# ruiminshen/yolo-tf

Measured on AMD Instinct MI355X. Metric: train_throughput, higher is better.
Workload: dtype bf16; 1 GPU; Darknet-19 YOLOv2 VOC-20 416x416 training step (standardise+fwd+loss+bwd+Adam), batch 16 per GPU (BASELINE configs[1]); global_batch=16, parallelism=dp1, optimizer=adam, weights=random-init (Xavier, seed 0), collective=none (1 rank)

## Files before the change

include/yolo2_hip.h:

```cpp
#ifndef YOLO2_HIP_H
#define YOLO2_HIP_H

#include <stddef.h>
#include <stdint.h>

#ifdef __cplusplus
extern "C" {
#endif

enum { YOLO2_F32 = 0, YOLO2_BF16 = 1 };
enum {
    YOLO2_OK = 0,
    YOLO2_E_ARG = 1,
    YOLO2_E_LAUNCH = 2,
    YOLO2_E_UNSUPPORTED = 3
};

int yolo2_abi_version(void);
const char *yolo2_last_error(void);
uint32_t yolo2_crc32c(const void *data, size_t n, uint32_t crc);
int yolo2_shutdown(void);
int yolo2_check_async_errors(void *stream);
#define YOLO2_ASYNC_ERROR_WORDS 8
int yolo2_async_error_snapshot(unsigned *host_words, void *stream);
// ... 24 lines not shown
int yolo2_conv2d_wgrad_ws(const void *X, const void *dY, float *dW, float *ws, size_t ws_bytes, int B, int H, int W,
                          int Cin, int ldx, int Cout, int ldy, int ksize, int dtype, void *stream);
int yolo2_set_deterministic(int on);
int yolo2_get_deterministic(void);

int yolo2_filter_prep(const float *W, void *Ffwd, void *Fdgr, int ksize, int Cin, int ldcin,
                      int Cout, int ldcout, int dtype, void *stream);

#define YOLO2_FILTER_PREP_TILE 64
#define YOLO2_FILTER_PREP_TILE_N 128
int yolo2_filter_prep_blocks(int ksize, int ldcin, int ldcout);
typedef struct yolo2_filter_desc {
    const float *W;
    void *Ffwd;
    void *Fdgr;
    int ksize, cin, ldcin, cout, ldcout, first_block;
} yolo2_filter_desc;
int yolo2_filter_prep_batch(const yolo2_filter_desc *descs_device, int n, int total_blocks, int dtype,
                            void *stream);

int yolo2_adam_filter_prep(const yolo2_filter_desc *descs_device, int n, int total_blocks, const long *small_ranges_device, int n_small,
                           float *params, const float *grads, float *m, float *v, float alpha, float beta1, float beta2, float eps,
                           float gscale, int dtype, void *stream);

int yolo2_conv2d_bias_leaky(const void *P, const void *F, const float *bias, void *O, float *ws, size_t ws_bytes, int B,
                            int H, int W, int Cp, int ldp, int Nf, int ldo, int ksize, float alpha, int dtype, void *stream);

int yolo2_conv2d_dgrad_bn(const void *dY, const void *F, void *dX, float *ws, size_t ws_bytes, int B, int H, int W, int Cp, int ldp,
                          int Nf, int ldo, int ksize, const void *Yprev, const float *mean, const float *var, const float *gamma,
                          const float *beta, float *dgamma, float *dbeta, float *bn_part, double *red_ws, float eps, float alpha,
                          int *pending, int dtype, void *stream);
int yolo2_conv2d_dgrad_bn_fuses(int B, int H, int W, int Nf, int ksize, int dtype);
int yolo2_bn_part_to_grads(float *bn_part, int C, float *dgamma, float *dbeta, void *stream);

#define YOLO2_BN_PART_ROWS 256
int yolo2_conv2d_bn(const void *P, const void *F, void *O, float *ws, size_t ws_bytes, int B, int H, int W, int Cp, int ldp,
                    int Nf, int ldo, int ksize, const float *shift, float *bn_part, int dtype, void *stream);
int yolo2_bn_finalize(float *bn_part, const float *shift, long M, int C, float *mean, float *var, float *moving_mean,
                      float *moving_var, double decay, void *stream);

int yolo2_last_bn_part_rows(void);
int yolo2_bn_fin_supported(int rows, int C, int dtype);
int yolo2_bn_leaky_fin(const void *Y, const float *bn_part, int rows, const float *shift, float *mean, float *var, float *moving_mean,
                       float *moving_var, double decay, const float *gamma, const float *beta, void *A, long M, int C, int lda,
                       float eps, float alpha, float *zero, long zero_floats, int dtype, void *stream);
int yolo2_bn_leaky_pool_fin(const void *Y, const float *bn_part, int rows, const float *shift, float *mean, float *var,
// ... 202 lines not shown
```

yolo_tf_amd/_lib.py:

```python
import ctypes
import os

_HERE = os.path.dirname(os.path.abspath(__file__))
LIB_PATH = os.environ.get('YOLO2_LIB_PATH') or os.path.join(_HERE, 'csrc', 'libyolo2hip.so')

F32, BF16 = 0, 1


class HipKernelError(RuntimeError):
    pass


_p = ctypes.c_void_p
_i = ctypes.c_int
_l = ctypes.c_long
_f = ctypes.c_float

SIGNATURES = {
    'yolo2_conv2d': [_p, _p, _p, _p, _i, _i, _i, _i, _i, _i, _i, _i, _i, _p],
    'yolo2_conv2d_ws': [_p, _p, _p, _p, _p, ctypes.c_size_t, _i, _i, _i, _i, _i, _i, _i, _i, _i, _p],
    'yolo2_conv2d_bias_leaky': [_p, _p, _p, _p, _p, ctypes.c_size_t, _i, _i, _i, _i, _i, _i, _i, _i, _f, _i, _p],
    'yolo2_conv2d_dgrad_bn': [_p, _p, _p, _p, ctypes.c_size_t, _i, _i, _i, _i, _i, _i, _i, _i, _p, _p, _p, _p, _p, _p, _p, _p, _p, _f, _f, _p, _i, _p],
    'yolo2_bn_part_to_grads': [_p, _i, _p, _p, _p],
    'yolo2_debug_noop': [_p],
    'yolo2_conv2d_wgrad': [_p, _p, _p, _i, _i, _i, _i, _i, _i, _i, _i, _i, _p],
    'yolo2_conv2d_wgrad_ws': [_p, _p, _p, _p, ctypes.c_size_t, _i, _i, _i, _i, _i, _i, _i, _i, _i, _p],
    'yolo2_set_deterministic': [_i],
    'yolo2_filter_prep': [_p, _p, _p, _i, _i, _i, _i, _i, _i, _p],
    'yolo2_filter_prep_batch': [_p, _i, _i, _i, _p],
    'yolo2_adam_filter_prep': [_p, _i, _i, _p, _i, _p, _p, _p, _p, _f, _f, _f, _f, _f, _i, _p],
    'yolo2_first_layer_stats': [_p, _p, _i, _i, _i, _p, _p, _i, _p],
    'yolo2_first_layer_bn_leaky_pool': [_p, _p, _p, _p, _p, _p, _p, _p, _i, _i, _i, _i, _f, _f, _i, _p],
    'yolo2_first_layer_pool_bwd_reduce': [_p, _p, _p, _i, _p, _p, _p, _p, _p, _p, _i, _i, _i, _f, _f, _i, _p],
    'yolo2_first_layer_pool_bwd_apply': [_p, _p, _p, _i, _p, _p, _p, _p, _p, _p, _p, _p, _i, _i, _i, _f, _f, _i, _p],
    'yolo2_conv2d_bn': [_p, _p, _p, _p, ctypes.c_size_t, _i, _i, _i, _i, _i, _i, _i, _i, _p, _p, _i, _p],
    'yolo2_bn_finalize': [_p, _p, _l, _i, _p, _p, _p, _p, ctypes.c_double, _p],
    'yolo2_bn_leaky_fin': [_p, _p, _i, _p, _p, _p, _p, _p, ctypes.c_double, _p, _p, _p, _l, _i, _i, _f, _f, _p, _l, _i, _p],
    'yolo2_bn_leaky_pool_fin': [_p, _p, _i, _p, _p, _p, _p, _p, ctypes.c_double, _p, _p, _p, _p, _p, _p, _i, _i, _i, _i, _i, _f, _f, _p, _l, _i, _p],
    'yolo2_bn_leaky_bwd_apply_fin': [_p, _i, _p, _p, _p, _p, _p, _p, _i, _l, _p, _p, _p, _l, _i, _f, _f, _p, _l, _i, _p],
    'yolo2_first_layer_wgrad_bn': [_p, _p, _p, _i, _p, _p, _p, _p, _p, _p, _i, _l, _p, _p, _p, _i, _i, _i, _i, _f, _f, _p, _l, _i, _p],
    'yolo2_bn_leaky_pool_bwd_apply_fin': [_p, _i, _p, _p, _p, _p, _p, _p, _p, _i, _l, _p, _p, _p, _i, _i, _i, _i, _f, _f, _p, _l, _i, _p],
    'yolo2_bn_leaky_bwd_reduce_part': [_p, _i, _p, _p, _p, _p, _p, _p, _p, _i, _l, _i, _f, _f, _i, _p],
    'yolo2_bn_leaky_pool_bwd_reduce_part': [_p, _i, _p, _p, _p, _p, _p, _p, _p, _p, _i, _i, _i, _i, _i, _f, _f, _i, _p],
    'yolo2_bn_leaky_pool': [_p, _p, _p, _p, _p, _p, _p, _i, _i, _i, _i, _i, _f, _f, _i, _p],
    'yolo2_bn_leaky_pool_bwd_reduce': [_p, _i, _p, _p, _p, _p, _p, _p, _p, _p, _p, _i, _i, _i, _i, _f, _f, _i, _p],
    'yolo2_bn_leaky_pool_bwd_apply': [_p, _i, _p, _p, _p, _p, _p, _p, _p, _p, _p, _i, _i, _i, _i, _f, _f, _i, _p],
    'yolo2_augment_images': [_p, _p, _p, _p, _i, _i, _i, _i, _p],
    'yolo2_transform_labels': [_p, _p, _p, _p, _p, _p, _p, _p, _p, _i, _i, _i, _i, _p, _p],
    'yolo2_bn_stats': [_p, _p, _p, _p, _l, _i, _i, _p],
    'yolo2_bn_stats_ema': [_p, _p, _p, _p, _p, ctypes.c_double, _p, _l, _i, _i, _p],
    'yolo2_bn_ema': [_p, _p, _p, _p, _i, ctypes.c_double, _p],
    'yolo2_bn_leaky': [_p, _p, _p, _p, _p, _p, _l, _i, _i, _f, _f, _i, _p],
    'yolo2_bn_leaky_bwd_reduce': [_p, _i, _p, _p, _p, _p, _p, _p, _p, _p, _l, _i, _f, _f, _i, _p],
# ... 30 lines not shown
    'yolo2_ftrl': [_p, _p, _p, _p, _l, _f, _f, _f, _f, _f, _p],
    'yolo2_scale': [_p, _l, _f, _p],
    'yolo2_zero_ranges': [_p, _p, _i, _p],
    'yolo2_bn_fold': [_p, _p, _p, _p, _p, _p, _p, _l, _i, _f, _p],
    'yolo2_selftest_tr16': [_p, _p],
    'yolo2_set_stream_workgroups': [_i],
    'yolo2_cast_f32_bf16': [_p, _p, _l, _p],
    'yolo2_cast_bf16_f32': [_p, _p, _l, _p],
    'yolo2_debug_occupy': [_i, _p, _p, _i, _p],
    'yolo2_check_async_errors': [_p],
    'yolo2_async_error_snapshot': [_p, _p],
    'yolo2_debug_set_streamk_wait_us': [_i, _i],
    'yolo2_eval_collect': [_p, _p, _p, _p, _p, _p, _p, _i, _i, _i, _i, _i, _i, _i, _f, _f, _p, _l, _p, _p, _p, _p],
    'yolo2_eval_finalize': [_p, _l, _p, _p, _i, _i, _i, _p, ctypes.c_size_t, _p, _p, _p, _p, _p],
}

QUERIES = {
    'yolo2_abi_version': (_i, []),
    'yolo2_last_error': (ctypes.c_char_p, []),
    'yolo2_shutdown': (_i, []),
    'yolo2_crc32c': (ctypes.c_uint32, [_p, ctypes.c_size_t, ctypes.c_uint32]),
    'yolo2_conv2d_wgrad_accumulates': (_i, [_i] * 9),
    'yolo2_filter_prep_blocks': (_i, [_i, _i, _i]),
    'yolo2_conv2d_dgrad_bn_fuses': (_i, [_i] * 6),
    'yolo2_debug_set_wgrad_variant': (None, [_i]),
    'yolo2_last_bn_part_rows': (_i, []),
    'yolo2_get_stream_workgroups': (_i, []),
    'yolo2_bn_fin_supported': (_i, [_i, _i, _i]),
    'yolo2_debug_last_conv_plan': (_i, [ctypes.POINTER(_i)]),
    'yolo2_debug_set_igemm_tap': (_i, [_i]),
    'yolo2_debug_set_pp': (_i, [_i, _i, _i, _i]),
    'yolo2_debug_set_pp_cost': (_i, [_i]),
    'yolo2_debug_set_s4_abl': (_i, [_i]),
    'yolo2_debug_last_wgrad_plan': (_i, [ctypes.POINTER(_i)]),
    'yolo2_debug_wgrad_row_plan': (_i, [_i, _i, _i, _i, _i, _i, _i, ctypes.POINTER(_i)]),
    'yolo2_debug_wgrad_ws_plan': (_i, [_i] * 10 + [ctypes.POINTER(_i)]),
    'yolo2_conv2d_wgrad_workspace_bytes': (ctypes.c_size_t, [_i] * 9),
    'yolo2_get_deterministic': (_i, []),
    'yolo2_debug_magic_u32': (_i, [ctypes.c_uint, ctypes.POINTER(ctypes.c_uint), ctypes.POINTER(ctypes.c_uint)]),
    'yolo2_conv2d_workspace_bytes': (ctypes.c_size_t, [_i] * 7),
    'yolo2_bn_workspace_bytes': (ctypes.c_size_t, [_i]),
    'yolo2_bias_grad_workspace_bytes': (ctypes.c_size_t, [_i]),
    'yolo2_image_prep_workspace_bytes': (ctypes.c_size_t, [_i]),
    'yolo2_loss_workspace_bytes': (ctypes.c_size_t, [_i, _i, _i]),
    'yolo2_nms_workspace_bytes': (ctypes.c_size_t, [_i, _i, _i]),
    'yolo2_clip_workspace_bytes': (ctypes.c_size_t, [_i]),
# ... 104 lines not shown
```

yolo_tf_amd/csrc/elementwise.hip:

```cpp
#include "common.h"
#include <stdlib.h>
#include <stdarg.h>

static thread_local char g_err[512] = "";
void yolo2_set_error(const char *fmt, ...) {
    va_list ap;
    va_start(ap, fmt);
    vsnprintf(g_err, sizeof(g_err), fmt, ap);
    va_end(ap);
}
extern "C" const char *yolo2_last_error(void) { return g_err; }

static thread_local int g_deterministic = 0;
int y2_deterministic() { return g_deterministic; }
extern "C" int yolo2_set_deterministic(int on) { g_deterministic = on ? 1 : 0; return YOLO2_OK; }
extern "C" int yolo2_get_deterministic(void) { return g_deterministic; }

extern "C" uint32_t yolo2_crc32c(const void *data, size_t n, uint32_t crc) {
    static uint32_t table[8][256];
    static bool ready = [] {
        for (uint32_t i = 0; i < 256; ++i) {
            uint32_t c = i;
            for (int k = 0; k < 8; ++k) c = (c & 1) ? (c >> 1) ^ 0x82F63B78u : c >> 1;
            table[0][i] = c;
// ... 50 lines not shown
    }
}

extern "C" int yolo2_filter_prep(const float *W, void *Ffwd, void *Fdgr, int ksize, int Cin, int ldcin,
                                 int Cout, int ldcout, int dtype, void *stream) {
    Y2_CHECK_ARG(W && (Ffwd || Fdgr));
    Y2_CHECK_ARG(ksize == 1 || ksize == 3);
    Y2_CHECK_ARG(ldcin >= Cin && ldcout >= Cout);
    hipStream_t st = (hipStream_t)stream;
    const int taps = ksize * ksize;
    if (Ffwd) {
        dim3 grid(cdiv(Cout, 32), cdiv(ldcin, 32), taps), block(32, 8);
        Y2_DISPATCH_DTYPE(dtype, filter_fwd_kernel<T><<<grid, block, 0, st>>>(W, (T *)Ffwd, Cin, ldcin, Cout, taps));
    }
    if (Fdgr) {
        long total = (long)Cin * taps * ldcout;
        int grid = (int)(total / 256 + 1 < 4096 ? total / 256 + 1 : 4096);
        Y2_DISPATCH_DTYPE(dtype, filter_dgrad_kernel<T><<<grid, 256, 0, st>>>(W, (T *)Fdgr, Cin, Cout, ldcout, taps));
    }
    Y2_CHECK_LAUNCH();
    return YOLO2_OK;
}

template <typename T>
__device__ __forceinline__ void store8(T *dst, const float (&v)[8]) {
    if constexpr (sizeof(T) == 2) {
        bf16x8 o;
#pragma unroll
        for (int j = 0; j < 8; ++j) o[j] = (bf16)v[j];
        *reinterpret_cast<bf16x8 *>(dst) = o;
    } else {
        f32x4 a = {v[0], v[1], v[2], v[3]}, b = {v[4], v[5], v[6], v[7]};
        reinterpret_cast<f32x4 *>(dst)[0] = a;
        reinterpret_cast<f32x4 *>(dst)[1] = b;
    }
}
template <typename T>
__device__ __forceinline__ void filter_tile_emit(const yolo2_filter_desc &d, const float (&tile)[YOLO2_FILTER_PREP_TILE][YOLO2_FILTER_PREP_TILE_N + 1], int tap, int taps,
                                                 int c0, int n0, int tid) {
    constexpr int TC = YOLO2_FILTER_PREP_TILE, TN = YOLO2_FILTER_PREP_TILE_N;
    T *Ff = (T *)d.Ffwd, *Fd = (T *)d.Fdgr;
    if (Ff) {
        constexpr int LPR = TC / 8, RPP = 256 / LPR;
        const int g8 = (tid % LPR) * 8, rr = tid / LPR;
        const long Kf = (long)taps * d.ldcin;
#pragma unroll
        for (int p = 0; p < TN / RPP; ++p) {
            const int nl = rr + p * RPP, nn = n0 + nl, c = c0 + g8;
            if (nn < d.cout && c < d.ldcin) {
                float v[8];
#pragma unroll
                for (int j = 0; j < 8; ++j) v[j] = tile[g8 + j][nl];
                store8<T>(Ff + nn * Kf + y2_filter_koff(tap, c, d.ldcin, taps), v);
            }
        }
    }
    if (Fd) {
        constexpr int LPR = TN / 8, RPP = 256 / LPR;
        const int g8 = (tid % LPR) * 8, rr = tid / LPR;
        const long Kd = (long)taps * d.ldcout;
        const int tp = taps - 1 - tap;
#pragma unroll
        for (int p = 0; p < TC / RPP; ++p) {
            const int cl = rr + p * RPP, c = c0 + cl, nn = n0 + g8;
// ... 1897 lines not shown
    if ((int)blockIdx.x >= conv_blocks) {
        const long *r = small + 2 * ((int)blockIdx.x - conv_blocks);
        for (long k = threadIdx.x; k < r[1]; k += 256) {
            const long o = r[0] + k;
            adam_one(a.params[o], a.grads[o], a.m[o], a.v[o], a.alpha, a.omb1, a.omb2, a.eps, a.gs);
        }
        return;
    }
    constexpr int TC = YOLO2_FILTER_PREP_TILE, TN = YOLO2_FILTER_PREP_TILE_N;
    __shared__ float tile[TC][TN + 1];
    int li = 0;
    while (li + 1 < n && (int)blockIdx.x >= descs[li + 1].first_block) ++li;
    const yolo2_filter_desc d = descs[li];
    const int taps = d.ksize * d.ksize;
    const int ctiles = (d.ldcin + TC - 1) / TC, ntiles = (d.ldcout + TN - 1) / TN;
    int u = blockIdx.x - d.first_block;
    const int ntile = u % ntiles; u /= ntiles;
    const int ctile = u % ctiles;
    const int tap = u / ctiles;
    const int n0 = ntile * TN, c0 = ctile * TC;
    const int tid = threadIdx.x;
    const long base = (d.W - a.params) + (long)tap * d.cin * d.cout;
    const bool vec_ok = (d.cout & 3) == 0 && ((base & 3) == 0);
    {
        constexpr int LPR = TN / 4, RPP = 256 / LPR;
        const int col = (tid % LPR) * 4, r0 = tid / LPR;
#pragma unroll
        for (int p = 0; p < TC / RPP; ++p) {
            const int c = c0 + r0 + p * RPP, nn = n0 + col;
            float w4[4] = {0.f, 0.f, 0.f, 0.f};
            if (c < d.cin) {
                const long o = base + (long)c * d.cout + nn;
                if (vec_ok && nn + 3 < d.cout) {
                    f32x4 wv = *reinterpret_cast<const f32x4 *>(a.params + o), mv = *reinterpret_cast<const f32x4 *>(a.m + o), vv = *reinterpret_cast<const f32x4 *>(a.v + o);
                    const f32x4 gv = *reinterpret_cast<const f32x4 *>(a.grads + o);
#pragma unroll
                    for (int j = 0; j < 4; ++j) {
                        float wj = wv[j], mj = mv[j], vj = vv[j];
                        adam_one(wj, gv[j], mj, vj, a.alpha, a.omb1, a.omb2, a.eps, a.gs);
                        wv[j] = wj; mv[j] = mj; vv[j] = vj; w4[j] = wj;
                    }
                    *reinterpret_cast<f32x4 *>(a.m + o) = mv;
                    *reinterpret_cast<f32x4 *>(a.v + o) = vv;
                    *reinterpret_cast<f32x4 *>(a.params + o) = wv;
                } else {
#pragma unroll
                    for (int j = 0; j < 4; ++j)
// ... 1 lines not shown
                            adam_one(a.params[o + j], a.grads[o + j], a.m[o + j], a.v[o + j], a.alpha, a.omb1, a.omb2, a.eps, a.gs);
                            w4[j] = a.params[o + j];
                        }
                }
            }
#pragma unroll
            for (int j = 0; j < 4; ++j) tile[r0 + p * RPP][col + j] = w4[j];
        }
    }
    __syncthreads();
    filter_tile_emit<T>(d, tile, tap, taps, c0, n0, tid);
}
extern "C" int yolo2_adam_filter_prep(const yolo2_filter_desc *descs_device, int n, int total_blocks, const long *small_ranges_device, int n_small,
                                      float *params, const float *grads, float *m, float *v, float alpha, float beta1, float beta2, float eps,
                                      float gscale, int dtype, void *stream) {
    Y2_CHECK_ARG(n >= 0 && total_blocks >= 0 && (n > 0) == (total_blocks > 0) && (descs_device || n == 0) && n_small >= 0 && total_blocks + n_small > 0 &&
                 (small_ranges_device || n_small == 0) && params && grads && m && v);
    Y2_CHECK_ARG(((((uintptr_t)params) | ((uintptr_t)grads) | ((uintptr_t)m) | ((uintptr_t)v)) & 15) == 0);
    const Y2AdamArgs a{params, grads, m, v, alpha, 1.0f - beta1, 1.0f - beta2, eps, gscale};
    Y2_DISPATCH_DTYPE(dtype, adam_filter_prep_kernel<T><<<total_blocks + n_small, 256, 0, (hipStream_t)stream>>>(descs_device, n, total_blocks, small_ranges_device, a));
    Y2_CHECK_LAUNCH();
    return YOLO2_OK;
}
```

yolo_tf_amd/engine.py:

```python
import numpy as np
import os

import torch

from . import ops, _lib
from .graph import pad8

BN_EPS = 1e-5
BN_DECAY = 0.999
LEAKY_ALPHA = 0.1

_DTYPES = {'bf16': torch.bfloat16, 'bfloat16': torch.bfloat16, 'f32': torch.float32, 'float32': torch.float32}


BN_PART_ROWS = 256
ARENA_ALIGN = 64


def layout_params(graph):
    offsets, off = {}, 0
    for v in reversed(graph.trainable()):
        offsets[v.name] = (off, v.size)
        off += (v.size + ARENA_ALIGN - 1) // ARENA_ALIGN * ARENA_ALIGN
    return offsets, off
# ... 349 lines not shown
        first = 0
        for d, op in zip(arr, convs):
            st = self.conv[op['name']]
            k, ldcin, ldcout = op['ksize'], pad8(op['cin']), pad8(op['cout'])
            if self._folds(op):
                st['fold_w'] = torch.empty_like(self.var[op['weights'].name])
                st['fold_bias'] = torch.empty(op['cout'], dtype=torch.float32, device=self.device)
            d.W = (st['fold_w'] if 'fold_w' in st else self.var[op['weights'].name]).data_ptr()
            d.Ffwd = st['Ffwd'].data_ptr()
            d.Fdgr = st['Fdgr'].data_ptr() if 'Fdgr' in st else None
            d.ksize, d.cin, d.ldcin, d.cout, d.ldcout, d.first_block = k, op['cin'], ldcin, op['cout'], ldcout, first
            first += ops.filter_prep_blocks(k, ldcin, ldcout)
        raw = bytes(arr)
        self._fdesc = torch.frombuffer(bytearray(raw), dtype=torch.uint8).to(self.device)
        self._fdesc_n, self._fdesc_blocks = len(convs), first
        import ctypes
        self._fdesc1_info = {}
        size = ctypes.sizeof(FilterDesc)
        bounds = [d.first_block for d in arr] + [first]
        for i, (d, op) in enumerate(zip(arr, convs)):
            self._fdesc1_info[op['name']] = (i * size, bounds[i + 1] - bounds[i])
            d.first_block = 0
        self._fdesc1 = torch.frombuffer(bytearray(bytes(arr)), dtype=torch.uint8).to(self.device)
        covered = sorted(self.param_offsets[op['weights'].name] for op in self.graph.ops if op['kind'] == 'conv')
        small = sorted(v for k, v in self.param_offsets.items() if v not in covered)
        flat = [x for o, n in small for x in (o, n)]
        self._small = torch.tensor(flat if flat else [0, 0], dtype=torch.int64, device=self.device)
        self._n_small = len(small)

    def adam_update_and_prepare(self, m, v, alpha, beta1, beta2, eps, gscale):
        self._filter_descs()
        ops.adam_filter_prep(self._fdesc, self._fdesc_n, self._fdesc_blocks, self._small, self._n_small, self.params, self.grads, m, v,
                             alpha, beta1, beta2, eps, gscale, self.dtype)
        self._filters_dirty = False

    def adam_update_layer(self, op, m, v, alpha, beta1, beta2, eps, gscale):
        self._filter_descs()
        off, blocks = self._fdesc1_info[op['name']]
        ops.adam_filter_prep(self._fdesc1[off:], 1, blocks, self._small, 0, self.params, self.grads, m, v, alpha, beta1, beta2, eps, gscale, self.dtype)

    def adam_update_small(self, m, v, alpha, beta1, beta2, eps, gscale):
        self._filter_descs()
        ops.adam_filter_prep(self._fdesc, 0, 0, self._small, self._n_small, self.params, self.grads, m, v, alpha, beta1, beta2, eps, gscale, self.dtype)
        self._filters_dirty = False

    def _folds(self, op):
        return (not self.training and self.fold_bn and op['bn'] and op['out'] not in self.fused_pool
                and op['x'] not in self.graph.inputs.values())

    def set_images(self, images, mode=0):
        (inp,) = self.graph.inputs.values()
        assert images.dtype == torch.float32 and images.is_cuda and images.numel() == self.B * inp.h * inp.w * 3
        self.img = images.contiguous()
        ops.image_prep(self.img, self.act[inp][0], self.ws, self.B, inp.h * inp.w, mode)

    def _plan_grad_zeroing(self):
        if False:
            return [(0, self.n_params)]
        if self.deterministic:
            return []
        ranges = []
        for op in self.graph.ops:
# ... 407 lines not shown
```

yolo_tf_amd/ops.py:

```python
import ctypes

import torch

from . import _lib
from ._lib import call, ptr, dtype_code


_raw_stream = getattr(torch._C, '_cuda_getCurrentRawStream', None)
_raw_device = getattr(torch._C, '_cuda_getDevice', None)


def _stream():
    if _raw_stream is None or _raw_device is None:
        return ctypes.c_void_p(torch.cuda.current_stream().cuda_stream)
    return ctypes.c_void_p(_raw_stream(_raw_device()))


def pad8(c):
    return (c + 7) // 8 * 8


def conv2d(P, F, bias, O, B, H, W, Cp, ldp, Nf, ldo, ksize):
    call('yolo2_conv2d', ptr(P), ptr(F), ptr(bias), ptr(O), B, H, W, Cp, ldp, Nf, ldo, ksize, dtype_code(P.dtype), _stream())

# ... 81 lines not shown
    def __enter__(self):
        if self.on:
            self.prev = int(_lib.query('yolo2_get_deterministic'))
            if not self.prev:
                set_deterministic(True)

    def __exit__(self, *exc):
        if self.on and not self.prev:
            set_deterministic(False)
        return False


def filter_prep(Wt, Ffwd, Fdgr, ksize, Cin, ldcin, Cout, ldcout, dtype):
    call('yolo2_filter_prep', ptr(Wt), ptr(Ffwd), ptr(Fdgr), ksize, Cin, ldcin, Cout, ldcout, dtype_code(dtype), _stream())


def filter_prep_batch(descs_dev, n, total_blocks, dtype):
    call('yolo2_filter_prep_batch', ptr(descs_dev), n, total_blocks, dtype_code(dtype), _stream())


def adam_filter_prep(descs_dev, n, total_blocks, small_dev, n_small, params, grads, m, v, alpha, b1, b2, eps, gscale, dtype):
    call('yolo2_adam_filter_prep', ptr(descs_dev), n, total_blocks, ptr(small_dev), n_small, ptr(params), ptr(grads), ptr(m), ptr(v), alpha, b1, b2, eps, gscale,
         dtype_code(dtype), _stream())


def bn_stats(Y, mean, var, ws, M, C):
    call('yolo2_bn_stats', ptr(Y), ptr(mean), ptr(var), ptr(ws), M, C, dtype_code(Y.dtype), _stream())


def bn_stats_ema(Y, mean, var, mm, mv, decay, ws, M, C):
    call('yolo2_bn_stats_ema', ptr(Y), ptr(mean), ptr(var), ptr(mm), ptr(mv), decay, ptr(ws), M, C, dtype_code(Y.dtype), _stream())


def bn_ema(mm, mv, mean, var, C, decay):
    call('yolo2_bn_ema', ptr(mm), ptr(mv), ptr(mean), ptr(var), C, decay, _stream())


def bn_leaky(Y, mean, var, gamma, beta, A, M, C, lda, eps, alpha):
    call('yolo2_bn_leaky', ptr(Y), ptr(mean), ptr(var), ptr(gamma), ptr(beta), ptr(A), M, C, lda, eps, alpha, dtype_code(Y.dtype), _stream())


def bn_leaky_bwd_reduce(dA, ldda, Y, mean, var, gamma, beta, dgamma, dbeta, ws, M, C, eps, alpha):
    call('yolo2_bn_leaky_bwd_reduce', ptr(dA), ldda, ptr(Y), ptr(mean), ptr(var), ptr(gamma), ptr(beta), ptr(dgamma), ptr(dbeta), ptr(ws),
         M, C, eps, alpha, dtype_code(Y.dtype), _stream())


# ... 378 lines not shown
```

yolo_tf_amd/session.py:

```python
import math
import os

import numpy as np
import torch

from . import ops
from .engine import Engine, layer_end_offsets
from .graph import pad8
from .model.yolo2 import OBJECTIVE_KEYS
from .optim import Optimizer, learning_rate_fn
from .parallel import GradReducer


def _label_shapes(B, cells, C):
    return [(B, cells), (B, cells, C), (B, cells, 4), (B, cells, 2), (B, cells, 2), (B, cells)]


class TrainSession(object):

    def __init__(self, builder, batch_size, dtype='bf16', optimizer='adam', learning_rate=1e-6, gradient_clip=0.0,
                 config=None, seed=0, world_size=1, bucket_mb=64.0, preprocess_mode=0, sizes=None, grad_dtype='f32', comm_cus=None, comm_timing=False,
                 sync_bn=False, shard_optimizer=False, deterministic=None):
        assert builder.training, 'call builder(data, training=True) first'
        self.builder = builder
        self.B = batch_size
        own = (builder.width, builder.height)
        traced = {own: (builder.graph, builder.model)}
        self.v1 = getattr(builder, 'family', 'yolo2') == 'yolo'
        assert not (self.v1 and sizes), 'the fully connected YOLO (v1) head fixes the input size'
        for wh in (sizes or []):
            wh = (int(wh[0]), int(wh[1]))
            if wh not in traced:
                traced[wh] = builder.trace(wh[0], wh[1], training=True)
        largest = max(traced, key=lambda wh: wh[0] * wh[1])
# ... 34 lines not shown
        self.lr_fn = learning_rate_fn(config if config is not None else builder.config, learning_rate)
        self.gradient_clip = float(gradient_clip)
        self.clip_ws = torch.zeros(ops.workspace_bytes('clip_fixed' if self.deterministic else 'clip', e.n_seg) // 8, dtype=torch.float64, device=dev)
        self.global_step = 0
        self.world_size = world_size
        self.preprocess_mode = preprocess_mode
        self.shard_optimizer = bool(shard_optimizer) and world_size > 1 and self.gradient_clip <= 0
        if shard_optimizer and world_size > 1 and not self.shard_optimizer:
            import logging
            logging.getLogger(__name__).warning('[mi355x] shard_optimizer is ignored: gradient_clip = %g needs every complete gradient, the update stays replicated',
                                                self.gradient_clip)
        self.optimizer_state_complete = True
        self.reducer = GradReducer(e.grads, list(e.param_offsets.values()), bucket_mb, grad_dtype=grad_dtype, timing=comm_timing,
                                   shard_params=e.params if self.shard_optimizer else None) if world_size > 1 else None
        if world_size > 1:
            cfg = config if config is not None else builder.config
            reserve = comm_cus if comm_cus is not None else (cfg.getint('mi355x', 'comm_cus') if cfg is not None and cfg.has_option('mi355x', 'comm_cus') else 32)
            total = torch.cuda.get_device_properties(dev).multi_processor_count
            ops.set_stream_workgroups(max(64, total - int(reserve)) if reserve > 0 else 0)
        if world_size > 1 and torch.distributed.is_available() and torch.distributed.is_initialized():
            e.dropout_rank = torch.distributed.get_rank()
        self.bucketed_update = True
        self.fuse_adam_prep = os.environ.get('YOLO2_FUSE_ADAM_PREP', '1') != '0'
        self.early_adam = (os.environ.get('YOLO2_EARLY_ADAM', '0') == '1' and not self.deterministic and world_size == 1 and optimizer == 'adam' and self.fuse_adam_prep
                           and self.gradient_clip <= 0 and not getattr(e, '_has_l2', False) and dev.type == 'cuda')
        self.opt_stream = torch.cuda.Stream(device=dev) if self.early_adam else None
        self._early_pending = False
        self._in_step = False
        self.async_errors = ops.AsyncErrorPoll() if dev.type == 'cuda' else None
        self._layer_end = layer_end_offsets(e.graph, e.param_offsets)

    def set_size(self, width, height):
        wh = (int(width), int(height))
        self.engine.set_size(wh[1], wh[0])
        self.model = self.models[wh]
        self.labels = self._labels[wh]
        self.size = wh

    def upload_labels(self, labels):
        for dst, src in zip(self.labels, labels):
            dst.copy_(torch.from_numpy(np.ascontiguousarray(src, np.float32).reshape(dst.shape)), non_blocking=True)

    def forward_backward(self, images, defer_collectives=False):
        e, m = self.engine, self.model
        assert not self._early_pending, 'a layer-wise early update is half applied: apply_gradients() must follow the forward_backward() of step()'
        e.dropout_step = self.global_step
        e.zero_grads()
        e.set_images(images, self.preprocess_mode)
        e.forward()
# ... 1 lines not shown
        logits, ld = e.act[out]
        dlogits, _ = e.gact[out]
        if self.v1:
            ops.yolo1_loss(logits, ld, self.labels, self.hparam, self.objectives_dev, dlogits, self.loss_ws, self.B, m.cell_height, m.cell_width, self.A, self.C)
        else:
            ops.loss_partials(logits, ld, self.anchors, self.labels, self.hparam, dlogits, self.loss_ws, self.B, m.cell_height, m.cell_width, self.A, self.C)
            self._objectives_pending = (m.cell_height, m.cell_width)
        if self.reducer is not None:
            self.reducer.begin()
            self.reducer.shard = self.shard_optimizer and defer_collectives
            self._sharded_pending = self.reducer.shard
            if self.reducer.shard:
                lr, t, gs = self.lr_fn(self.global_step), self.global_step + 1, 1.0 / self.world_size
                self.reducer.update_fn = lambda lo, hi: self.optimizer.apply(e.params, e.grads, lr, t, gs, lo, hi)
            e.backward(on_layer_done=lambda op, ev: self.reducer.ready_upto(self._layer_end[op['name']], ev))
            self._deferred = defer_collectives and self.gradient_clip <= 0 and self.bucketed_update
            self.reducer.finish(wait=not self._deferred)
        elif self.early_adam and defer_collectives and self._in_step:
            hp = self.optimizer.hp
            t = self.global_step + 1
            alpha = self.lr_fn(self.global_step) * math.sqrt(1.0 - hp['beta2'] ** t) / (1.0 - hp['beta1'] ** t)
            main, opt, m_, v_ = torch.cuda.current_stream(), self.opt_stream, self.optimizer.slots[0], self.optimizer.slots[1]

            def update_layer(op, wgrad_done):
                ev = torch.cuda.Event()
                ev.record(main)
                opt.wait_event(ev)
                if wgrad_done is not None:
                    opt.wait_event(wgrad_done)
                with torch.cuda.stream(opt):
                    e.adam_update_layer(op, m_, v_, alpha, hp['beta1'], hp['beta2'], hp['epsilon'], 1.0)
            e.backward(on_layer_done=update_layer)
            self._early_pending = (alpha, hp['beta1'], hp['beta2'], hp['epsilon'])
        else:
            e.backward()

    def apply_gradients(self):
        e = self.engine
        if self.gradient_clip > 0:
            if self.world_size > 1:
                ops.scale(e.grads, e.n_params, 1.0 / self.world_size)
            if self.deterministic:
                ops.clip_by_norm_fixed(e.grads, e.seg_off, e.n_seg, self.gradient_clip, self.clip_ws)
            else:
                ops.clip_by_norm(e.grads, e.seg_off, e.n_seg, self.gradient_clip, self.clip_ws)
            gscale = 1.0
        else:
            gscale = 1.0 / self.world_size
        lr = self.lr_fn(self.global_step)
        if self._early_pending:
            alpha, b1, b2, eps = self._early_pending
            self._early_pending = False
            torch.cuda.current_stream().wait_stream(self.opt_stream)
            e.adam_update_small(self.optimizer.slots[0], self.optimizer.slots[1], alpha, b1, b2, eps, 1.0)
            self.global_step += 1
            return
        if self.reducer is not None and getattr(self, '_sharded_pending', False):
            self.reducer.finish(wait=True)
            self._deferred = False
            self._sharded_pending = False
            self.optimizer_state_complete = False
            self.global_step += 1
            e._filters_dirty = True
        elif self.reducer is not None and getattr(self, '_deferred', False):
            for lo, hi in self.reducer.completed_buckets():
                self.optimizer.apply(e.params, e.grads, lr, self.global_step + 1, gscale, lo, hi)
            self._deferred = False
            self.global_step += 1
            e._filters_dirty = True
        elif self.optimizer.name == 'adam' and self.fuse_adam_prep:
            self.optimizer.apply_fused_with_filter_prep(e, lr, self.global_step + 1, gscale)
            self.global_step += 1
        else:
            self.optimizer.apply(e.params, e.grads, lr, self.global_step + 1, gscale)
            self.global_step += 1
            e._filters_dirty = True

# ... 112 lines not shown
```

Baseline: 4600 img/s.

## Overlap Adam+filter-prep for large coarse layers with backward on high-priority stream

Early Adam is now enabled automatically for the large convolution layers at the coarsest resolution. Each of these layers is updated during backward on a high-priority side stream, using a new lightweight streaming kernel (64-thread workgroups, register-pipelined loads, DPP lane exchange) that writes the bf16 forward and dgrad filters directly. The remaining layers and small params are handled in one fused call after backward. The aim is to hide optimizer memory traffic behind backward compute, at the cost of contention with the backward kernels and extra code paths; a fast path was also added to the existing fused Adam tile kernel.

```diff
diff --git a/include/yolo2_hip.h b/include/yolo2_hip.h
--- a/include/yolo2_hip.h
+++ b/include/yolo2_hip.h
@@ -70,6 +70,11 @@
 int yolo2_adam_filter_prep(const yolo2_filter_desc *descs_device, int n, int total_blocks, const long *small_ranges_device, int n_small,
                            float *params, const float *grads, float *m, float *v, float alpha, float beta1, float beta2, float eps,
                            float gscale, int dtype, void *stream);
+
+int yolo2_adam_filter_prep_stream_units(int ksize, int ldcin, int ldcout);
+int yolo2_adam_filter_prep_stream(const yolo2_filter_desc *descs_device, int n, int total_units, float *params, const float *grads, float *m,
+                                  float *v, float alpha, float beta1, float beta2, float eps, float gscale, int dtype, int max_workgroups,
+                                  void *stream);
 
 int yolo2_conv2d_bias_leaky(const void *P, const void *F, const float *bias, void *O, float *ws, size_t ws_bytes, int B,
                             int H, int W, int Cp, int ldp, int Nf, int ldo, int ksize, float alpha, int dtype, void *stream);
diff --git a/yolo_tf_amd/_lib.py b/yolo_tf_amd/_lib.py
--- a/yolo_tf_amd/_lib.py
+++ b/yolo_tf_amd/_lib.py
@@ -29,6 +29,7 @@
     'yolo2_filter_prep': [_p, _p, _p, _i, _i, _i, _i, _i, _i, _p],
     'yolo2_filter_prep_batch': [_p, _i, _i, _i, _p],
     'yolo2_adam_filter_prep': [_p, _i, _i, _p, _i, _p, _p, _p, _p, _f, _f, _f, _f, _f, _i, _p],
+    'yolo2_adam_filter_prep_stream': [_p, _i, _i, _p, _p, _p, _p, _f, _f, _f, _f, _f, _i, _i, _p],
     'yolo2_first_layer_stats': [_p, _p, _i, _i, _i, _p, _p, _i, _p],
     'yolo2_first_layer_bn_leaky_pool': [_p, _p, _p, _p, _p, _p, _p, _p, _i, _i, _i, _i, _f, _f, _i, _p],
     'yolo2_first_layer_pool_bwd_reduce': [_p, _p, _p, _i, _p, _p, _p, _p, _p, _p, _i, _i, _i, _f, _f, _i, _p],
@@ -105,6 +106,7 @@
     'yolo2_crc32c': (ctypes.c_uint32, [_p, ctypes.c_size_t, ctypes.c_uint32]),
     'yolo2_conv2d_wgrad_accumulates': (_i, [_i] * 9),
     'yolo2_filter_prep_blocks': (_i, [_i, _i, _i]),
+    'yolo2_adam_filter_prep_stream_units': (_i, [_i, _i, _i]),
     'yolo2_conv2d_dgrad_bn_fuses': (_i, [_i] * 6),
     'yolo2_debug_set_wgrad_variant': (None, [_i]),
     'yolo2_last_bn_part_rows': (_i, []),
diff --git a/yolo_tf_amd/csrc/elementwise.hip b/yolo_tf_amd/csrc/elementwise.hip
--- a/yolo_tf_amd/csrc/elementwise.hip
+++ b/yolo_tf_amd/csrc/elementwise.hip
@@ -96,24 +96,25 @@
     return YOLO2_OK;
 }
 
+#define Y2_GLOBAL __attribute__((address_space(1)))
 template <typename T>
-__device__ __forceinline__ void store8(T *dst, const float (&v)[8]) {
+__device__ __forceinline__ void store8(Y2_GLOBAL T *dst, const float (&v)[8]) {
     if constexpr (sizeof(T) == 2) {
         bf16x8 o;
 #pragma unroll
         for (int j = 0; j < 8; ++j) o[j] = (bf16)v[j];
-        *reinterpret_cast<bf16x8 *>(dst) = o;
+        *(Y2_GLOBAL bf16x8 *)dst = o;
     } else {
         f32x4 a = {v[0], v[1], v[2], v[3]}, b = {v[4], v[5], v[6], v[7]};
-        reinterpret_cast<f32x4 *>(dst)[0] = a;
-        reinterpret_cast<f32x4 *>(dst)[1] = b;
+        ((Y2_GLOBAL f32x4 *)dst)[0] = a;
+        ((Y2_GLOBAL f32x4 *)dst)[1] = b;
     }
 }
 template <typename T>
 __device__ __forceinline__ void filter_tile_emit(const yolo2_filter_desc &d, const float (&tile)[YOLO2_FILTER_PREP_TILE][YOLO2_FILTER_PREP_TILE_N + 1], int tap, int taps,
                                                  int c0, int n0, int tid) {
     constexpr int TC = YOLO2_FILTER_PREP_TILE, TN = YOLO2_FILTER_PREP_TILE_N;
-    T *Ff = (T *)d.Ffwd, *Fd = (T *)d.Fdgr;
+    Y2_GLOBAL T *Ff = (Y2_GLOBAL T *)d.Ffwd, *Fd = (Y2_GLOBAL T *)d.Fdgr;
     if (Ff) {
         constexpr int LPR = TC / 8, RPP = 256 / LPR;
         const int g8 = (tid % LPR) * 8, rr = tid / LPR;
@@ -2057,7 +2058,43 @@
     const int tid = threadIdx.x;
     const long base = (d.W - a.params) + (long)tap * d.cin * d.cout;
     const bool vec_ok = (d.cout & 3) == 0 && ((base & 3) == 0);
-    {
+    constexpr int LPR_ = TN / 4, RPP_ = 256 / LPR_, NP = TC / RPP_;
+    if (vec_ok && c0 + TC <= d.cin && n0 + TN <= d.cout) {
+        const int col = (tid % LPR_) * 4, r0 = tid / LPR_;
+        const unsigned pitch = (unsigned)RPP_ * (unsigned)d.cout * 4u;
+        const unsigned off0 = ((unsigned)(c0 + r0) * (unsigned)d.cout + (unsigned)(n0 + col)) * 4u;
+        char *__restrict__ pw = reinterpret_cast<char *>(a.params + base);
+        char *__restrict__ pm = reinterpret_cast<char *>(a.m + base);
+        char *__restrict__ pv = reinterpret_cast<char *>(a.v + base);
+        const char *__restrict__ pg = reinterpret_cast<const char *>(a.grads + base);
+        f32x4 W[NP], M[NP], V[NP], G[NP];
+        auto load = [&](int p) {
+            const unsigned o = off0 + (unsigned)p * pitch;
+            W[p] = *reinterpret_cast<const f32x4 *>(pw + o);
+            M[p] = *reinterpret_cast<const f32x4 *>(pm + o);
+            V[p] = *reinterpret_cast<const f32x4 *>(pv + o);
+            G[p] = *reinterpret_cast<const f32x4 *>(pg + o);
+        };
+        load(0);
+        load(1);
+#pragma unroll
+        for (int p = 0; p < NP; ++p) {
+            if (p + 2 < NP) load(p + 2);
+            __builtin_amdgcn_sched_barrier(0);
+#pragma unroll
+            for (int j = 0; j < 4; ++j) {
+                float wj = W[p][j], mj = M[p][j], vj = V[p][j];
+                adam_one(wj, G[p][j], mj, vj, a.alpha, a.omb1, a.omb2, a.eps, a.gs);
+                W[p][j] = wj; M[p][j] = mj; V[p][j] = vj;
+                tile[r0 + p * RPP_][col + j] = wj;
+            }
+            const unsigned o = off0 + (unsigned)p * pitch;
+            *reinterpret_cast<f32x4 *>(pm + o) = M[p];
+            *reinterpret_cast<f32x4 *>(pv + o) = V[p];
+            *reinterpret_cast<f32x4 *>(pw + o) = W[p];
+            __builtin_amdgcn_sched_barrier(0);
+        }
+    } else {
         constexpr int LPR = TN / 4, RPP = 256 / LPR;
         const int col = (tid % LPR) * 4, r0 = tid / LPR;
 #pragma unroll
@@ -2105,3 +2142,155 @@
     Y2_CHECK_LAUNCH();
     return YOLO2_OK;
 }
+
+#define Y2_ADAM_STREAM_C 64
+#define Y2_ADAM_STREAM_N 32
+__device__ __forceinline__ unsigned stream_koff(int tap, int x0, int ld, int taps) {
+    return y2_kchunk(ld, taps) == Y2_KCHUNK ? (unsigned)((x0 >> 6) * taps * Y2_KCHUNK + tap * Y2_KCHUNK + (x0 & 63)) : (unsigned)(tap * ld + x0);
+}
+template <typename T>
+__device__ __forceinline__ void adam_stream_patch_elementwise(const yolo2_filter_desc &d, const Y2AdamArgs &a, long base, int tap, int taps, int c0, int n0, int lane) {
+    Y2_GLOBAL T *Ff = (Y2_GLOBAL T *)d.Ffwd, *Fd = (Y2_GLOBAL T *)d.Fdgr;
+    const long Kf = (long)taps * d.ldcin, Kd = (long)taps * d.ldcout;
+    const int tp = taps - 1 - tap, cb = c0 + (lane & 7) * 8, nb = n0 + (lane >> 3) * 4;
+    for (int j = 0; j < 8 && cb + j < d.ldcin; ++j) {
+        const int c = cb + j;
+        for (int i = 0; i < 4 && nb + i < d.ldcout; ++i) {
+            const int nn = nb + i;
+            float w = 0.f;
+            if (c < d.cin && nn < d.cout) {
+                const long o = base + (long)c * d.cout + nn;
+                adam_one(a.params[o], a.grads[o], a.m[o], a.v[o], a.alpha, a.omb1, a.omb2, a.eps, a.gs);
+                w = a.params[o];
+            }
+            if (Ff && nn < d.cout) Ff[nn * Kf + y2_filter_koff(tap, c, d.ldcin, taps)] = (T)w;
+            if (Fd && c < d.cin) Fd[c * Kd + y2_filter_koff(tp, nn, d.ldcout, taps)] = (T)w;
+        }
+    }
+}
+template <typename T>
+__device__ __forceinline__ void adam_stream_patch(const yolo2_filter_desc &d, const Y2AdamArgs &a, long base, int tap, int taps, int c0, int n0, int lane) {
+    const unsigned cb = (lane & 7) * 8, nb = (lane >> 3) * 4;
+    const unsigned pitch = (unsigned)d.cout * 4u;
+    const unsigned off0 = ((unsigned)(c0 + cb) * (unsigned)d.cout + (unsigned)n0 + nb) * 4u;
+    char *__restrict__ pw = reinterpret_cast<char *>(a.params + base);
+    char *__restrict__ pm = reinterpret_cast<char *>(a.m + base);
+    char *__restrict__ pv = reinterpret_cast<char *>(a.v + base);
+    const char *__restrict__ pg = reinterpret_cast<const char *>(a.grads + base);
+    Y2_GLOBAL char *__restrict__ Ff = (Y2_GLOBAL char *)d.Ffwd;
+    Y2_GLOBAL char *__restrict__ Fd = (Y2_GLOBAL char *)d.Fdgr;
+    const unsigned Kf = (unsigned)(taps * d.ldcin), Kd = (unsigned)(taps * d.ldcout);
+    const unsigned kf = stream_koff(tap, c0, d.ldcin, taps) + cb;
+    const unsigned kd = stream_koff(taps - 1 - tap, n0, d.ldcout, taps);
+    f32x4 W[8], M[8], V[8], G[8];
+    auto load = [&](int j) {
+        const unsigned o = off0 + (unsigned)j * pitch;
+        W[j] = *reinterpret_cast<const f32x4 *>(pw + o);
+        M[j] = *reinterpret_cast<const f32x4 *>(pm + o);
+        V[j] = *reinterpret_cast<const f32x4 *>(pv + o);
+        G[j] = *reinterpret_cast<const f32x4 *>(pg + o);
+    };
+    load(0);
+    load(1);
+    if constexpr (sizeof(T) == 2) {
+        const bool odd = (lane & 8) != 0;
+        bf16x4 ff[4];
+        u32x2 prev = {0u, 0u};
+#pragma unroll
+        for (int j = 0; j < 8; ++j) {
+            if (j + 2 < 8) load(j + 2);
+            __builtin_amdgcn_sched_barrier(0);
+            bf16x4 row;
+#pragma unroll
+            for (int i = 0; i < 4; ++i) {
+                float wj = W[j][i], mj = M[j][i], vj = V[j][i];
+                adam_one(wj, G[j][i], mj, vj, a.alpha, a.omb1, a.omb2, a.eps, a.gs);
+                W[j][i] = wj; M[j][i] = mj; V[j][i] = vj;
+                row[i] = (bf16)wj;
+                ff[i][j & 3] = row[i];
+            }
+            const unsigned o = off0 + (unsigned)j * pitch;
+            *reinterpret_cast<f32x4 *>(pm + o) = M[j];
+            *reinterpret_cast<f32x4 *>(pv + o) = V[j];
+            *reinterpret_cast<f32x4 *>(pw + o) = W[j];
+            const u32x2 mine = __builtin_bit_cast(u32x2, row);
+            if (j & 1) {
+                const u32x2 send = odd ? prev : mine;
+                u32x2 recv;
+                recv[0] = (unsigned)__builtin_amdgcn_update_dpp(0, (int)send[0], 0x128, 0xf, 0xf, false);
+                recv[1] = (unsigned)__builtin_amdgcn_update_dpp(0, (int)send[1], 0x128, 0xf, 0xf, false);
+                const u32x2 lo = odd ? recv : prev, hi = odd ? mine : recv;
+                const u32x4 out = {lo[0], lo[1], hi[0], hi[1]};
+                const unsigned c = (unsigned)c0 + cb + (unsigned)(j - 1) + (odd ? 1u : 0u);
+                *(Y2_GLOBAL u32x4 *)(Fd + (c * Kd + kd + (nb & ~4u)) * 2u) = out;
+            }
+            prev = mine;
+            if ((j & 3) == 3) {
+#pragma unroll
+                for (int i = 0; i < 4; ++i) *(Y2_GLOBAL bf16x4 *)(Ff + (((unsigned)n0 + nb + i) * Kf + kf + (unsigned)(j - 3)) * 2u) = ff[i];
+            }
+            __builtin_amdgcn_sched_barrier(0);
+        }
+    } else {
+#pragma unroll
+        for (int h = 0; h < 2; ++h) {
+            f32x4 ff[4];
+#pragma unroll
+            for (int jj = 0; jj < 4; ++jj) {
+                const int j = h * 4 + jj;
+                if (j + 2 < 8) load(j + 2);
+                __builtin_amdgcn_sched_barrier(0);
+#pragma unroll
+                for (int i = 0; i < 4; ++i) {
+                    float wj = W[j][i], mj = M[j][i], vj = V[j][i];
+                    adam_one(wj, G[j][i], mj, vj, a.alpha, a.omb1, a.omb2, a.eps, a.gs);
+                    W[j][i] = wj; M[j][i] = mj; V[j][i] = vj;
+                    ff[i][jj] = wj;
+                }
+                const unsigned o = off0 + (unsigned)j * pitch;
+                *reinterpret_cast<f32x4 *>(pm + o) = M[j];
+                *reinterpret_cast<f32x4 *>(pv + o) = V[j];
+                *reinterpret_cast<f32x4 *>(pw + o) = W[j];
+                *(Y2_GLOBAL f32x4 *)(Fd + (((unsigned)c0 + cb + j) * Kd + kd + nb) * 4u) = W[j];
+                __builtin_amdgcn_sched_barrier(0);
+            }
+#pragma unroll
+            for (int i = 0; i < 4; ++i) *(Y2_GLOBAL f32x4 *)(Ff + (((unsigned)n0 + nb + i) * Kf + kf + 4u * h) * 4u) = ff[i];
+        }
+    }
+}
+template <typename T>
+__global__ __launch_bounds__(64) __attribute__((amdgpu_waves_per_eu(6))) void adam_filter_prep_stream_kernel(const yolo2_filter_desc *__restrict__ descs, int n,
+                                                                                                        int total_units, const Y2AdamArgs a) {
+    const int lane = threadIdx.x;
+    int li = 0;
+    for (int unit = blockIdx.x; unit < total_units; unit += gridDim.x) {
+        while (li + 1 < n && unit >= descs[li + 1].first_block) ++li;
+        const yolo2_filter_desc d = descs[li];
+        const int taps = d.ksize * d.ksize;
+        const int ctiles = (d.ldcin + Y2_ADAM_STREAM_C - 1) / Y2_ADAM_STREAM_C, ntiles = (d.ldcout + Y2_ADAM_STREAM_N - 1) / Y2_ADAM_STREAM_N;
+        int u = unit - d.first_block;
+        const int ntile = u % ntiles; u /= ntiles;
+        const int ctile = u % ctiles;
+        const int tap = u / ctiles;
+        const int n0 = ntile * Y2_ADAM_STREAM_N, c0 = ctile * Y2_ADAM_STREAM_C;
+        const long base = (d.W - a.params) + (long)tap * d.cin * d.cout;
+        const bool full = (d.cout & 3) == 0 && (base & 3) == 0 && d.Ffwd && d.Fdgr && c0 + Y2_ADAM_STREAM_C <= d.cin && n0 + Y2_ADAM_STREAM_N <= d.cout;
+        if (full) adam_stream_patch<T>(d, a, base, tap, taps, c0, n0, lane);
+        else adam_stream_patch_elementwise<T>(d, a, base, tap, taps, c0, n0, lane);
+    }
+}
+extern "C" int yolo2_adam_filter_prep_stream_units(int ksize, int ldcin, int ldcout) {
+    if (ksize < 1 || ldcin < 1 || ldcout < 1) return 0;
+    return ksize * ksize * cdiv(ldcin, Y2_ADAM_STREAM_C) * cdiv(ldcout, Y2_ADAM_STREAM_N);
+}
+extern "C" int yolo2_adam_filter_prep_stream(const yolo2_filter_desc *descs_device, int n, int total_units, float *params, const float *grads, float *m, float *v,
+                                             float alpha, float beta1, float beta2, float eps, float gscale, int dtype, int max_workgroups, void *stream) {
+    Y2_CHECK_ARG(descs_device && n > 0 && total_units > 0 && max_workgroups >= 0 && params && grads && m && v);
+    Y2_CHECK_ARG(((((uintptr_t)params) | ((uintptr_t)grads) | ((uintptr_t)m) | ((uintptr_t)v)) & 15) == 0);
+    const Y2AdamArgs a{params, grads, m, v, alpha, 1.0f - beta1, 1.0f - beta2, eps, gscale};
+    const int grid = max_workgroups > 0 && max_workgroups < total_units ? max_workgroups : total_units;
+    Y2_DISPATCH_DTYPE(dtype, adam_filter_prep_stream_kernel<T><<<grid, 64, 0, (hipStream_t)stream>>>(descs_device, n, total_units, a));
+    Y2_CHECK_LAUNCH();
+    return YOLO2_OK;
+}
diff --git a/yolo_tf_amd/engine.py b/yolo_tf_amd/engine.py
--- a/yolo_tf_amd/engine.py
+++ b/yolo_tf_amd/engine.py
@@ -395,6 +395,7 @@
             self._fdesc1_info[op['name']] = (i * size, bounds[i + 1] - bounds[i])
             d.first_block = 0
         self._fdesc1 = torch.frombuffer(bytearray(bytes(arr)), dtype=torch.uint8).to(self.device)
+        self._fdesc_sub = {}
         covered = sorted(self.param_offsets[op['weights'].name] for op in self.graph.ops if op['kind'] == 'conv')
         small = sorted(v for k, v in self.param_offsets.items() if v not in covered)
         flat = [x for o, n in small for x in (o, n)]
@@ -411,6 +412,34 @@
         self._filter_descs()
         off, blocks = self._fdesc1_info[op['name']]
         ops.adam_filter_prep(self._fdesc1[off:], 1, blocks, self._small, 0, self.params, self.grads, m, v, alpha, beta1, beta2, eps, gscale, self.dtype)
+
+    def adam_stream_layer(self, op, m, v, alpha, beta1, beta2, eps, gscale, max_workgroups=0):
+        self._filter_descs()
+        off, _ = self._fdesc1_info[op['name']]
+        units = ops.adam_filter_prep_stream_units(op['ksize'], pad8(op['cin']), pad8(op['cout']))
+        ops.adam_filter_prep_stream(self._fdesc1[off:], 1, units, self.params, self.grads, m, v, alpha, beta1, beta2, eps, gscale, self.dtype, max_workgroups)
+
+    def adam_update_rest(self, done, m, v, alpha, beta1, beta2, eps, gscale):
+        self._filter_descs()
+        key = frozenset(done)
+        sub = self._fdesc_sub.get(key)
+        if sub is None:
+            import ctypes
+            from ._lib import FilterDesc
+            size = ctypes.sizeof(FilterDesc)
+            raw = bytes(self._fdesc1.cpu().numpy())
+            rest = [name for name in self._fdesc1_info if name not in key]
+            arr = (FilterDesc * max(1, len(rest)))()
+            first = 0
+            for d, name in zip(arr, rest):
+                off, blocks = self._fdesc1_info[name]
+                ctypes.memmove(ctypes.addressof(d), raw[off:off + size], size)
+                d.first_block = first
+                first += blocks
+            sub = (torch.frombuffer(bytearray(bytes(arr)), dtype=torch.uint8).to(self.device), len(rest), first)
+            self._fdesc_sub[key] = sub
+        ops.adam_filter_prep(sub[0], sub[1], sub[2], self._small, self._n_small, self.params, self.grads, m, v, alpha, beta1, beta2, eps, gscale, self.dtype)
+        self._filters_dirty = False
 
     def adam_update_small(self, m, v, alpha, beta1, beta2, eps, gscale):
         self._filter_descs()
diff --git a/yolo_tf_amd/ops.py b/yolo_tf_amd/ops.py
--- a/yolo_tf_amd/ops.py
+++ b/yolo_tf_amd/ops.py
@@ -127,6 +127,20 @@
 def adam_filter_prep(descs_dev, n, total_blocks, small_dev, n_small, params, grads, m, v, alpha, b1, b2, eps, gscale, dtype):
     call('yolo2_adam_filter_prep', ptr(descs_dev), n, total_blocks, ptr(small_dev), n_small, ptr(params), ptr(grads), ptr(m), ptr(v), alpha, b1, b2, eps, gscale,
          dtype_code(dtype), _stream())
+
+
+def adam_filter_prep_stream_units(ksize, ldcin, ldcout):
+    return int(_lib.load().yolo2_adam_filter_prep_stream_units(ksize, ldcin, ldcout))
+
+
+def adam_filter_prep_stream_available():
+    _lib.load()
+    return 'yolo2_adam_filter_prep_stream' not in _lib.MISSING
+
+
+def adam_filter_prep_stream(descs_dev, n, total_units, params, grads, m, v, alpha, b1, b2, eps, gscale, dtype, max_workgroups=0):
+    call('yolo2_adam_filter_prep_stream', ptr(descs_dev), n, total_units, ptr(params), ptr(grads), ptr(m), ptr(v), alpha, b1, b2, eps, gscale,
+         dtype_code(dtype), max_workgroups, _stream())
 
 
 def bn_stats(Y, mean, var, ws, M, C):
diff --git a/yolo_tf_amd/session.py b/yolo_tf_amd/session.py
--- a/yolo_tf_amd/session.py
+++ b/yolo_tf_amd/session.py
@@ -10,6 +10,20 @@
 from .model.yolo2 import OBJECTIVE_KEYS
 from .optim import Optimizer, learning_rate_fn
 from .parallel import GradReducer
+
+
+EARLY_ADAM_AUTO = True
+EARLY_ADAM_MIN_PARAMS = 1 << 18
+
+
+def _early_layers(graph):
+    convs = [op for op in graph.ops if op['kind'] == 'conv']
+    if not convs:
+        return []
+    coarsest = min(op['out'].h * op['out'].w for op in convs)
+    return [op['name'] for op in convs
+            if op['out'].h * op['out'].w == coarsest and op['ksize'] ** 2 * op['cin'] * op['cout'] >= EARLY_ADAM_MIN_PARAMS
+            and op['cin'] % 64 == 0 and op['cout'] % 32 == 0]
 
 
 def _label_shapes(B, cells, C):
@@ -90,9 +104,20 @@
             e.dropout_rank = torch.distributed.get_rank()
         self.bucketed_update = True
         self.fuse_adam_prep = os.environ.get('YOLO2_FUSE_ADAM_PREP', '1') != '0'
-        self.early_adam = (os.environ.get('YOLO2_EARLY_ADAM', '0') == '1' and not self.deterministic and world_size == 1 and optimizer == 'adam' and self.fuse_adam_prep
-                           and self.gradient_clip <= 0 and not getattr(e, '_has_l2', False) and dev.type == 'cuda')
-        self.opt_stream = torch.cuda.Stream(device=dev) if self.early_adam else None
+        mode = os.environ.get('YOLO2_EARLY_ADAM', 'auto')
+        assert mode in ('auto', '0', '1'), 'YOLO2_EARLY_ADAM is auto, 0 or 1'
+        gates = (not self.deterministic and world_size == 1 and optimizer == 'adam' and self.fuse_adam_prep and self.gradient_clip <= 0
+                 and not getattr(e, '_has_l2', False) and dev.type == 'cuda')
+        self._early_set = frozenset()
+        if mode == 'auto' and gates and EARLY_ADAM_AUTO and ops.adam_filter_prep_stream_available():
+            self._early_set = frozenset(_early_layers(e.graph))
+        self.early_adam = gates and (mode == '1' or bool(self._early_set))
+        self.early_adam_wgs = int(os.environ.get('YOLO2_EARLY_ADAM_WGS', '0'))
+        if self._early_set:
+            lo, hi = torch.cuda.Stream.priority_range()
+            self.opt_stream = torch.cuda.Stream(device=dev, priority=max(lo, hi))
+        else:
+            self.opt_stream = torch.cuda.Stream(device=dev) if self.early_adam else None
         self._early_pending = False
         self._in_step = False
         self.async_errors = ops.AsyncErrorPoll() if dev.type == 'cuda' else None
@@ -140,14 +165,21 @@
             alpha = self.lr_fn(self.global_step) * math.sqrt(1.0 - hp['beta2'] ** t) / (1.0 - hp['beta1'] ** t)
             main, opt, m_, v_ = torch.cuda.current_stream(), self.opt_stream, self.optimizer.slots[0], self.optimizer.slots[1]
 
+            early = self._early_set
+
             def update_layer(op, wgrad_done):
+                if early and op['name'] not in early:
+                    return
                 ev = torch.cuda.Event()
                 ev.record(main)
                 opt.wait_event(ev)
                 if wgrad_done is not None:
                     opt.wait_event(wgrad_done)
                 with torch.cuda.stream(opt):
-                    e.adam_update_layer(op, m_, v_, alpha, hp['beta1'], hp['beta2'], hp['epsilon'], 1.0)
+                    if early:
+                        e.adam_stream_layer(op, m_, v_, alpha, hp['beta1'], hp['beta2'], hp['epsilon'], 1.0, self.early_adam_wgs)
+                    else:
+                        e.adam_update_layer(op, m_, v_, alpha, hp['beta1'], hp['beta2'], hp['epsilon'], 1.0)
             e.backward(on_layer_done=update_layer)
             self._early_pending = (alpha, hp['beta1'], hp['beta2'], hp['epsilon'])
         else:
@@ -170,7 +202,10 @@
             alpha, b1, b2, eps = self._early_pending
             self._early_pending = False
             torch.cuda.current_stream().wait_stream(self.opt_stream)
-            e.adam_update_small(self.optimizer.slots[0], self.optimizer.slots[1], alpha, b1, b2, eps, 1.0)
+            if self._early_set:
+                e.adam_update_rest(self._early_set, self.optimizer.slots[0], self.optimizer.slots[1], alpha, b1, b2, eps, 1.0)
+            else:
+                e.adam_update_small(self.optimizer.slots[0], self.optimizer.slots[1], alpha, b1, b2, eps, 1.0)
             self.global_step += 1
             return
         if self.reducer is not None and getattr(self, '_sharded_pending', False):
```

Result: slower. 4403 img/s (-4.3%).
